# dangvansam/viet-asr

Hardware: AMD Instinct MI355X
Metric: real_time_factor (higher is better)
Workload: dtype f32 via 2xf16 split operands (22-bit significands, 3 f16 MFMA products per multiply, fp32 accumulate); 1 GPU; BASELINE configs[2]: quartznet15x5 greedy CTC, batch=64x10s 16kHz mono per GPU, wav in HBM -> collapsed ids; batch_per_gpu=64, parallelism=utterance-shard x1

## Files before the change

include/vasr_devtools.h:

```cpp
#ifndef VASR_DEVTOOLS_H_
#define VASR_DEVTOOLS_H_
#include "vasr.h"
#ifdef __cplusplus
extern "C" {
#endif

VASR_API int vasr_profile_bracket_overhead(vasr_stream stream, int n, double* out_us);
VASR_API int vasr_fused_tile_choice(int64_t tiles128, int compute_units);
VASR_API int vasr_bench_depthwise(const float* d_x, const float* d_w, const int32_t* d_lens, int batch, int channels,
                         int64_t frames, int kernel, float* d_y, vasr_stream stream);
VASR_API int vasr_bench_depthwise_layer(const float* d_x, const float* d_w, const int32_t* d_lens_in, const int32_t* d_lens_out,
                               int batch, int channels, int64_t frames_in, int kernel, int stride, int dilation, float* d_y,
                               uint32_t* d_amax, int amax_stride, vasr_stream stream);
VASR_API int vasr_depthwise_mfma_table_size(int kernel, int dilation);
VASR_API int vasr_pack_depthwise_taps(const float* h_w, int channels, int kernel, int dilation, uint32_t* h_table, float* h_inv);
VASR_API int vasr_bench_depthwise_mfma(const float* d_x, const uint32_t* d_taps, const float* d_tap_inv, const int32_t* d_lens,
                              int batch, int channels, int64_t frames, int kernel, int dilation, float* d_y,
                              uint32_t* d_amax, int amax_stride, vasr_stream stream);
VASR_API int vasr_pack_pointwise(const float* h_w, int cout, int cin, int m_pad, float* h_out);
VASR_API int vasr_conv_gemm_weights(const float* h_w, int cout, int cin, int kernel, float* h_out);
VASR_API int vasr_bench_pointwise(const float* d_x, const float* d_wt, const float* d_scale, const float* d_shift,
                         int batch, int cin, int cout, int64_t frames, float* d_y, vasr_stream stream);

VASR_API int vasr_bench_mfma_sustained(int gemm_mode, int workgroups, int steps, float* d_sink, double* flops, vasr_stream stream);
// ... 18 lines not shown
```

viet-asr_amd/_lib.py:

```python
import ctypes as C
import os

import numpy as np
import torch

_HERE = os.path.dirname(os.path.abspath(__file__))
LIB_PATH = os.environ.get("VASR_LIB_PATH") or os.path.join(_HERE, "lib", "libvasr_hip.so")
DEV_LIB_PATH = os.environ.get("VASR_LIB_PATH") or os.path.join(_HERE, "lib", "libvasr_hip_dev.so")


class VasrError(RuntimeError):
    pass


class BlockDesc(C.Structure):
    _fields_ = [(n, C.c_int32) for n in
                ("filters", "repeat", "kernel", "stride", "dilation", "residual", "separable", "residual_dense")]


class FrontendDesc(C.Structure):
    _fields_ = [("sample_rate", C.c_int32), ("n_fft", C.c_int32), ("win_length", C.c_int32),
                ("hop_length", C.c_int32), ("n_mels", C.c_int32), ("preemph", C.c_float),
                ("log_guard", C.c_float), ("normalize", C.c_int32),
                ("h_window", C.POINTER(C.c_float)), ("h_filterbank", C.POINTER(C.c_float)),
# ... 63 lines not shown
    "vasr_algorithmic_work": (C.c_int, [_P, C.c_int, C.c_int64, C.POINTER(C.c_double)]),
    "vasr_profile_begin": (C.c_int, [_P]),
    "vasr_profile_end": (C.c_int, [_P, C.POINTER(C.c_double), C.POINTER(C.c_int64), C.POINTER(C.c_double), C.POINTER(C.c_double)]),
    "vasr_padded_frames": (C.c_int64, [C.c_int64]),
}

DEV_SIGNATURES = {
    "vasr_pack_pointwise_f16x2": (C.c_int, [_P, C.c_int, C.c_int, C.c_int, _P, C.POINTER(C.c_float)]),
    "vasr_bench_pointwise_f16x2": (C.c_int, [_P, _P, C.c_float, _P, _P, C.c_int, C.c_int, C.c_int, C.c_int64, _P, _P,
                                             C.c_int, _P]),
    "vasr_depthwise_mfma_table_size": (C.c_int, [C.c_int, C.c_int]),
    "vasr_pack_depthwise_taps": (C.c_int, [_P, C.c_int, C.c_int, C.c_int, _P, _P]),
    "vasr_bench_depthwise_mfma": (C.c_int, [_P, _P, _P, _P, C.c_int, C.c_int, C.c_int64, C.c_int, C.c_int, _P, _P, C.c_int, _P]),
    "vasr_profile_bracket_overhead": (C.c_int, [_P, C.c_int, C.POINTER(C.c_double)]),
    "vasr_fused_tile_choice": (C.c_int, [C.c_int64, C.c_int]),
    "vasr_pack_pointwise": (C.c_int, [_P, C.c_int, C.c_int, C.c_int, _P]),
    "vasr_conv_gemm_weights": (C.c_int, [_P, C.c_int, C.c_int, C.c_int, _P]),
    "vasr_pack_pointwise_bf16x3": (C.c_int, [_P, C.c_int, C.c_int, C.c_int, _P]),
    "vasr_bench_pointwise_bf16x3": (C.c_int, [_P, _P, _P, _P, C.c_int, C.c_int, C.c_int, C.c_int64, _P, _P]),
    "vasr_bench_mfma_sustained": (C.c_int, [C.c_int, C.c_int, C.c_int, _P, C.POINTER(C.c_double), _P]),
    "vasr_bench_depthwise": (C.c_int, [_P, _P, _P, C.c_int, C.c_int, C.c_int64, C.c_int, _P, _P]),
    "vasr_bench_depthwise_layer": (C.c_int, [_P, _P, _P, _P, C.c_int, C.c_int, C.c_int64, C.c_int, C.c_int, C.c_int, _P, _P,
                                             C.c_int, _P]),
    "vasr_bench_pointwise": (C.c_int, [_P, _P, _P, _P, C.c_int, C.c_int, C.c_int, C.c_int64, _P, _P]),
    "vasr_bench_groupnorm": (C.c_int, [_P, _P, C.c_int, C.c_int, C.c_int64, C.c_int, C.c_int, _P, _P, C.c_int, _P, _P]),
}

ABI_VERSION = 8

_lib = None
# ... 175 lines not shown
```

viet-asr_amd/csrc/frontend.hip:

```cpp
#include <atomic>

#include "vasr_internal.h"
#include "len_chain.h"
#include "vasr_device.h"

namespace vasr {

namespace {

constexpr int kWaves = 8;
constexpr int kThreads = 64 * kWaves;
constexpr int kNfft = 512;

struct cf { float re, im; };
__device__ __forceinline__ cf cadd(cf a, cf b) { return {a.re + b.re, a.im + b.im}; }
__device__ __forceinline__ cf csub(cf a, cf b) { return {a.re - b.re, a.im - b.im}; }
__device__ __forceinline__ cf cmul(cf a, cf b) { return {a.re * b.re - a.im * b.im, a.re * b.im + a.im * b.re}; }
__device__ __forceinline__ cf cmul_negi(cf a) { return {a.im, -a.re}; }


__device__ __forceinline__ float sample_f32(const float* x, int64_t n) { return x[n]; }
__device__ __forceinline__ float sample_f32(const short* x, int64_t n) { return (float)x[n] * 0x1p-15f; }

template <int kFramesPerBlock, typename S>
__global__ __launch_bounds__(kThreads, 4) void stft_logmel_kernel(FrontendTables tb, const S* __restrict__ wav,
                                                          int64_t samples, const int64_t* __restrict__ row_len,
                                                          int hop, float preemph,
                                                          float log_guard, float* __restrict__ mel,
                                                          int64_t mel_ld, int frames) {
  constexpr int kFramesPerWave = kFramesPerBlock / kWaves;
  extern __shared__ __attribute__((aligned(16))) float smem[];
  const int seg_len = (kFramesPerBlock - 1) * hop + kNfft;
  float* seg = smem;
  cf* fftbuf = reinterpret_cast<cf*>(seg + ((seg_len + 3) & ~3));
  float* pbuf = reinterpret_cast<float*>(fftbuf + kWaves * 256);
  float* tile = pbuf + kWaves * (260 + kMelTaps);

  const int tid = threadIdx.x, lane = tid & 63, wave = tid >> 6;
  const int b = blockIdx.y;
  const int f0 = blockIdx.x * kFramesPerBlock;
  const S* x = wav + (int64_t)b * samples;
  const int64_t ns = row_len ? min(row_len[b], samples) : samples;

  const float2* win2 = reinterpret_cast<const float2*>(tb.window);
  const float2* t256 = reinterpret_cast<const float2*>(tb.tw256);
  const float2* t512 = reinterpret_cast<const float2*>(tb.tw512);
  float2 wn[4];
#pragma unroll
  for (int r = 0; r < 4; ++r) wn[r] = win2[lane + 64 * r];
  cf tws[3][3];
#pragma unroll
  for (int g = 0; g < 3; ++g) {
    const int Ns = 4 << (2 * g), step = (lane & (Ns - 1)) * (64 / Ns);
#pragma unroll
    for (int m = 0; m < 3; ++m) { const float2 w = t256[(m + 1) * step]; tws[g][m] = {w.x, w.y}; }
  }
  cf twk[5];
#pragma unroll
  for (int i = 0; i < 5; ++i) { const float2 w = t512[min(lane + 64 * i, 256)]; twk[i] = {w.x, w.y}; }
  const int64_t p0 = (int64_t)f0 * hop - kNfft / 2;
  for (int i = tid; i < seg_len; i += kThreads) {
    int64_t n = p0 + i;
    if (n < 0) n = -n;
    if (n >= ns) n = 2 * (ns - 1) - n;
    float v = 0.f;
    if (n >= 0 && n < ns) {
      v = sample_f32(x, n);
      if (preemph >= 0.f && n > 0) v = __fsub_rn(v, __fmul_rn(preemph, sample_f32(x, n - 1)));
    }
    seg[i] = v;
  }
  float mw[kMelTaps];
#pragma unroll
  for (int i = 0; i < kMelTaps; ++i) mw[i] = tb.mel_w[lane * kMelTaps + i];
  const int mlo = tb.mel_lo[lane];
  float* P = pbuf + wave * (260 + kMelTaps);
  for (int i = lane; i < 260 + kMelTaps; i += 64) P[i] = 0.f;
  __syncthreads();

  cf* buf = fftbuf + wave * 256;

  for (int jf = 0; jf < kFramesPerWave; ++jf) {
    const int fl = wave * kFramesPerWave + jf;
    const float* s = seg + fl * hop;
    {
      cf v[4];
#pragma unroll
      for (int r = 0; r < 4; ++r) {
        const int q = lane + 64 * r;
        v[r] = {s[2 * q] * wn[r].x, s[2 * q + 1] * wn[r].y};
      }
      cf t0 = cadd(v[0], v[2]), t1 = csub(v[0], v[2]), t2 = cadd(v[1], v[3]), t3 = cmul_negi(csub(v[1], v[3]));
      buf[4 * lane + 0] = cadd(t0, t2);
      buf[4 * lane + 1] = cadd(t1, t3);
      buf[4 * lane + 2] = csub(t0, t2);
      buf[4 * lane + 3] = csub(t1, t3);
    }
    wave_fence();
#pragma unroll
    for (int g = 0; g < 3; ++g) {
      const int Ns = 4 << (2 * g);
      const int k = lane & (Ns - 1);
      cf v[4];
#pragma unroll
      for (int r = 0; r < 4; ++r) v[r] = buf[lane + 64 * r];
      wave_fence();
      v[1] = cmul(v[1], tws[g][0]);
      v[2] = cmul(v[2], tws[g][1]);
      v[3] = cmul(v[3], tws[g][2]);
      cf t0 = cadd(v[0], v[2]), t1 = csub(v[0], v[2]), t2 = cadd(v[1], v[3]), t3 = cmul_negi(csub(v[1], v[3]));
      const int j0 = (lane / Ns) * Ns * 4 + k;
      buf[j0] = cadd(t0, t2);
      buf[j0 + Ns] = cadd(t1, t3);
      buf[j0 + 2 * Ns] = csub(t0, t2);
      buf[j0 + 3 * Ns] = csub(t1, t3);
      wave_fence();
    }
    const cf* Z = buf;
#pragma unroll
    for (int i = 0; i < 5; ++i) {
      const int k = lane + 64 * i;
      if (k > 256) break;
      cf zk = Z[k & 255];
      cf zc = Z[(256 - k) & 255];
      zc.im = -zc.im;
      cf e = {0.5f * (zk.re + zc.re), 0.5f * (zk.im + zc.im)};
      cf d = {zk.re - zc.re, zk.im - zc.im};
      cf o = {0.5f * d.im, -0.5f * d.re};
      cf xk = cadd(e, cmul(twk[i], o));
      P[k] = xk.re * xk.re + xk.im * xk.im;
    }
    wave_fence();
    float acc = 0.f;
#pragma unroll
    for (int i = 0; i < kMelTaps; ++i) acc = fmaf(mw[i], P[mlo + i], acc);
    tile[lane * (kFramesPerBlock + 1) + fl] = tb.guard_clamp ? logf(fmaxf(acc, log_guard)) : logf(acc + log_guard);
    wave_fence();
  }
  __syncthreads();
  for (int idx = tid; idx < 64 * kFramesPerBlock; idx += kThreads) {
    const int f = idx / kFramesPerBlock, j = idx % kFramesPerBlock;
    const int t = f0 + j;
    if (t < frames) mel[((int64_t)b * 64 + f) * mel_ld + t] = tile[f * (kFramesPerBlock + 1) + j];
  }
}

__global__ void seq_len_kernel(const int64_t* __restrict__ len, int batch, int hop, int64_t* __restrict__ seq) {
  const int b = blockIdx.x * blockDim.x + threadIdx.x;
  if (b < batch) seq[b] = (int64_t)ceilf((float)len[b] / (float)hop);
}

__device__ __forceinline__ double wave_sum(double v) {
#pragma unroll
  for (int o = 32; o > 0; o >>= 1) v += __shfl_xor(v, o, 64);
  return v;
}

__device__ __forceinline__ int64_t seq_of(int64_t len, int hop) { return (int64_t)ceilf((float)len / (float)hop); }

constexpr int kRowsPerWg = 4;
__device__ __forceinline__ void normalize_row(float* __restrict__ x, int n, int frames, int normalize, double* red) {
  const int tid = threadIdx.x & 255, lane = tid & 63, wv = tid >> 6;
  float mean = 0.f, stdv = 1.f;
  if (normalize) {
    double s = 0.0;
    for (int t = tid; t < n; t += 256) s += (double)x[t];
    s = wave_sum(s);
    if (lane == 0) red[wv] = s;
    __syncthreads();
    const double mu = (((red[0] + red[1]) + red[2]) + red[3]) / (double)n;
    double q = 0.0;
    for (int t = tid; t < n; t += 256) { const double d = (double)x[t] - mu; q += d * d; }
    q = wave_sum(q);
    if (lane == 0) red[4 + wv] = q;
    __syncthreads();
    mean = (float)mu;
    stdv = (float)sqrt((((red[4] + red[5]) + red[6]) + red[7]) / (double)(n - 1));
    stdv = stdv + 1e-5f;
  }
  for (int t = tid; t < frames; t += 256) {
    float v = 0.f;
    if (t < n) v = normalize ? (x[t] - mean) / stdv : x[t];
    x[t] = v;
  }
}

__global__ __launch_bounds__(256 * kRowsPerWg) void normalize_kernel(float* __restrict__ mel, int64_t ld,
                                                                     const int64_t* __restrict__ seq, int rows, int n_mels,
                                                                     int frames, int normalize) {
  __shared__ double red[kRowsPerWg][8];
  const int grp = threadIdx.x >> 8;
  const int row = min((int)blockIdx.x * kRowsPerWg + grp, rows - 1);
  const int64_t n64 = seq[row / n_mels];
  normalize_row(mel + (int64_t)row * ld, (int)(n64 < 0 ? 0 : (n64 > frames ? frames : n64)), frames, normalize, red[grp]);
}

__global__ __launch_bounds__(256) void normalize_all_kernel(float* __restrict__ mel, int64_t ld, const int64_t* __restrict__ seq,
                                                            int n_mels, int frames) {
  __shared__ double red[8];
  const int tid = threadIdx.x, lane = tid & 63, wv = tid >> 6;
  float* x = mel + (int64_t)blockIdx.x * n_mels * ld;
  const int64_t n64 = seq[blockIdx.x];
  const int n = (int)(n64 < 0 ? 0 : (n64 > frames ? frames : n64));
  const double cnt = (double)n * (double)n_mels;
  double s = 0.0;
  for (int f = 0; f < n_mels; ++f)
    for (int t = tid; t < n; t += 256) s += (double)x[(int64_t)f * ld + t];
  s = wave_sum(s);
  if (lane == 0) red[wv] = s;
// ... 4 lines not shown
    for (int t = tid; t < n; t += 256) { const double d = (double)x[(int64_t)f * ld + t] - mu; q += d * d; }
  q = wave_sum(q);
  if (lane == 0) red[4 + wv] = q;
  __syncthreads();
  const float mean = (float)mu;
  const float stdv = (float)sqrt((((red[4] + red[5]) + red[6]) + red[7]) / (cnt - 1.0)) + 1e-5f;
  for (int f = 0; f < n_mels; ++f)
    for (int t = tid; t < n; t += 256) x[(int64_t)f * ld + t] = (x[(int64_t)f * ld + t] - mean) / stdv;
}

__global__ __launch_bounds__(256 * kRowsPerWg) void normalize_chain_kernel(float* __restrict__ mel, int64_t ld,
                                                              const int64_t* __restrict__ len, int hop, int batch, int n_mels,
                                                              int frames, int normalize, int64_t* __restrict__ seq,
                                                              const LenStep* __restrict__ steps, int n_steps,
                                                              int32_t* __restrict__ lens_tab, float* __restrict__ enc_len,
                                                              const int64_t* __restrict__ wav_len, int frames_cap) {
  __shared__ double red[kRowsPerWg][8];
  const int rows = batch * n_mels, row_wgs = (rows + kRowsPerWg - 1) / kRowsPerWg;
  if ((int)blockIdx.x < row_wgs) {
    const int grp = threadIdx.x >> 8;
    const int row = min((int)blockIdx.x * kRowsPerWg + grp, rows - 1);
    const int64_t n64 = seq_of(len[row / n_mels], hop);
    normalize_row(mel + (int64_t)row * ld, (int)(n64 < 0 ? 0 : (n64 > frames ? frames : n64)), frames, normalize, red[grp]);
    return;
  }
  const int b = ((int)blockIdx.x - row_wgs) * 256 * kRowsPerWg + (int)threadIdx.x;
  const int64_t l0 = b < batch ? seq_of(len[b], hop) : 0;
  if (b < batch) seq[b] = l0;
  len_chain_body(b, l0, batch, steps, n_steps, lens_tab, enc_len, wav_len, hop, frames_cap);
}

}

void launch_stft_logmel(const FrontendTables& tb, const void* wav, bool pcm16, int batch, int64_t samples,
                        const int64_t* row_len, int hop, float preemph, float log_guard, float* mel, int64_t mel_ld, int frames,
                        hipStream_t st) {
  auto go = [&](auto kern, auto* wav, int fpb) {
    const int seg_len = (fpb - 1) * hop + kNfft;
    const size_t lds = (size_t)((seg_len + 3) & ~3) * 4 + kWaves * 256 * 8 + kWaves * (260 + kMelTaps) * 4 + 64 * (fpb + 1) * 4;
    dim3 grid((frames + fpb - 1) / fpb, batch);
    hipLaunchKernelGGL(kern, grid, dim3(kThreads), lds, st, tb, wav, samples, row_len, hop, preemph, log_guard, mel, mel_ld,
                       frames);
  };
  const bool small = (int64_t)((frames + 31) / 32) * batch < 128;
  if (pcm16) {
    if (small) go(stft_logmel_kernel<8, short>, static_cast<const short*>(wav), 8);
    else go(stft_logmel_kernel<32, short>, static_cast<const short*>(wav), 32);
  } else {
    if (small) go(stft_logmel_kernel<8, float>, static_cast<const float*>(wav), 8);
    else go(stft_logmel_kernel<32, float>, static_cast<const float*>(wav), 32);
  }
}

void launch_seq_len(const int64_t* len, int batch, int hop, int64_t* seq, hipStream_t st) {
  hipLaunchKernelGGL(seq_len_kernel, dim3((batch + 63) / 64), dim3(64), 0, st, len, batch, hop, seq);
}

constexpr int kAloneLds = 152 * 1024;

void launch_normalize_all(float* mel, int64_t mel_ld, const int64_t* seq, int batch, int n_mels, int frames, hipStream_t st) {
  static std::atomic<uint64_t> opted{0};
  (void)dyn_lds_opt_in(reinterpret_cast<const void*>(normalize_all_kernel), kAloneLds, opted);
  hipLaunchKernelGGL(normalize_all_kernel, dim3(batch), dim3(256), kAloneLds, st, mel, mel_ld, seq, n_mels, frames);
}

void launch_normalize(float* mel, int64_t mel_ld, const int64_t* seq, int batch, int n_mels, int frames,
                      int normalize, hipStream_t st) {
  const int rows = batch * n_mels;
  static std::atomic<uint64_t> opted{0};
  (void)dyn_lds_opt_in(reinterpret_cast<const void*>(normalize_kernel), kAloneLds, opted);
  hipLaunchKernelGGL(normalize_kernel, dim3((rows + kRowsPerWg - 1) / kRowsPerWg), dim3(256 * kRowsPerWg), normalize ? kAloneLds : 0, st, mel, mel_ld,
                     seq, rows, n_mels, frames, normalize);
}

void launch_normalize_chain(float* mel, int64_t mel_ld, const int64_t* len, int hop, int batch, int n_mels, int frames,
                            int normalize, int64_t* seq, const LenStep* d_steps, int n_steps, int32_t* lens_tab,
                            float* enc_len, const int64_t* wav_len, int frames_cap, hipStream_t st) {
  const int rows = batch * n_mels;
  static std::atomic<uint64_t> opted{0};
  (void)dyn_lds_opt_in(reinterpret_cast<const void*>(normalize_chain_kernel), kAloneLds, opted);
  const int wg = 256 * kRowsPerWg;
  hipLaunchKernelGGL(normalize_chain_kernel, dim3((rows + kRowsPerWg - 1) / kRowsPerWg + (batch + wg - 1) / wg), dim3(wg), normalize ? kAloneLds : 0, st, mel, mel_ld, len, hop, batch,
                     n_mels, frames, normalize, seq, d_steps, n_steps, lens_tab, enc_len, wav_len, frames_cap);
}

}
```

viet-asr_amd/csrc/vasr_api.cpp:

```cpp
#include <hip/hip_runtime.h>

#include <cmath>
#include <cstdarg>
#include <cstdio>
#include <cstdlib>
#include <cstring>
#include <map>
#include <memory>
#include <string>
#include <algorithm>
#include <vector>

#include "vasr.h"
#include "vasr_host.h"
#include "vasr_internal.h"

using namespace vasr;

namespace {
thread_local std::string g_err;
}

namespace vasr {

// ... 1321 lines not shown
  return whole;
}

int vasr_melspec_f32(vasr_handle* h, const float* d_wav, const int64_t* d_len, int batch, int64_t samples,
                     float* d_mel, int64_t* d_seq, vasr_stream stream) {
  if (!h || !h->has_frontend || !h->finalized) return fail(VASR_ERR_STATE, "no finalized front end in this handle");
  if (batch <= 0 || !d_wav || !d_len || !d_mel || !d_seq) return fail(VASR_ERR_INVALID, "bad argument");
  if (samples <= h->fe.n_fft / 2)
    return fail(VASR_ERR_INVALID, "reflect padding needs more than n_fft/2 = %d samples (got %lld)",
                h->fe.n_fft / 2, (long long)samples);
  hipStream_t st = static_cast<hipStream_t>(stream);
  const int T = (int)vasr_mel_frames(h, samples);
  launch_seq_len(d_len, batch, h->fe.hop_length, d_seq, st);
  launch_stft_logmel(h->ft, d_wav, false, batch, samples, h->row_independent ? d_len : nullptr, h->fe.hop_length,
                     h->fe.preemph, h->fe.log_guard, d_mel, T, T, st);
  launch_normalize(d_mel, T, d_seq, batch, h->fe.n_mels, T, h->fe.normalize == 1, st);
  if (h->fe.normalize == 2) launch_normalize_all(d_mel, T, d_seq, batch, h->fe.n_mels, T, st);
  return check_launch("melspec");
}

int vasr_encoder_f32(vasr_handle* h, const float* d_mel, const int64_t* d_seq, int batch, int64_t mel_frames,
                     float* d_enc, float* d_enc_len, void* d_ws, size_t ws_bytes, vasr_stream stream) {
  if (!h || !h->has_encoder || !h->finalized) return fail(VASR_ERR_STATE, "no finalized encoder in this handle");
  if (batch <= 0 || mel_frames <= 0 || !d_mel || !d_seq || !d_enc || !d_ws) return fail(VASR_ERR_INVALID, "bad argument");
  const WsPlan p = plan_ws(h, batch, mel_frames);
  if (ws_bytes < p.total) return fail(VASR_ERR_WORKSPACE, "workspace %zu < %zu bytes", ws_bytes, p.total);
  hipStream_t st = static_cast<hipStream_t>(stream);
  char* ws = static_cast<char*>(d_ws);
  const Block& b0 = h->blocks[0];
  if (b0.subs[0].separable && !b0.has_res)
    return run_encoder(h, d_mel, mel_frames, mel_frames, d_seq, batch, d_enc, p.T1, d_enc_len, ws, p, st);
// ... 131 lines not shown

static int transcribe_part(vasr_handle* h, const void* d_wav, bool pcm16, const int64_t* d_len, int batch, int64_t samples,
                           int64_t* d_pred, int32_t* d_ids, int32_t* d_id_len, float* d_logp, float* d_enc_len,
                           char* ws, hipStream_t st) {
  const int64_t T = vasr_mel_frames(h, samples);
  const WsPlan p = plan_ws(h, batch, T);
  int64_t* seq = reinterpret_cast<int64_t*>(ws + p.seq);
  float* melp = reinterpret_cast<float*>(ws + p.melp);
  float* encp = reinterpret_cast<float*>(ws + p.encp);
  float* logits = reinterpret_cast<float*>(ws + p.logits);
  int64_t* pred = d_pred ? d_pred : reinterpret_cast<int64_t*>(ws + p.pred);
  {
    ProfScope ps(h, kProfFrontend, st);
    launch_stft_logmel(h->ft, d_wav, pcm16, batch, samples, h->row_independent ? d_len : nullptr, h->fe.hop_length,
                       h->fe.preemph, h->fe.log_guard, melp, p.Tp0, (int)T, st);
    launch_normalize_chain(melp, p.Tp0, d_len, h->fe.hop_length, batch, h->fe.n_mels, (int)T, h->fe.normalize == 1, seq,
                           h->d_steps, (int)h->steps.size(), reinterpret_cast<int32_t*>(ws + p.lens_tab), d_enc_len,
                           h->row_independent ? d_len : nullptr, (int)p.T1, st);
    if (h->fe.normalize == 2) launch_normalize_all(melp, p.Tp0, seq, batch, h->fe.n_mels, (int)T, st);
  }
  AmaxTab enc_amax{};
  const int32_t* own_frames = nullptr;
  int rc = run_encoder(h, melp, p.Tp0, T, seq, batch, encp, p.Tp1, d_enc_len, ws, p, st, &enc_amax, d_len, &own_frames, true);
  if (rc) return rc;
  if ((rc = run_decoder(h, encp, p.Tp1, p.T1, batch, logits, d_logp, pred, st, enc_amax, own_frames))) return rc;
  if (d_ids && d_id_len) {
    ProfScope ps(h, kProfHead, st);
    if (h->row_independent)
      launch_ctc_collapse(pred, batch, p.T1, h->num_classes - 1, d_ids, d_id_len, st, d_len, h->fe.hop_length,
                          h->d_steps, (int)h->steps.size());
    else
      launch_ctc_collapse(pred, batch, p.T1, h->num_classes - 1, d_ids, d_id_len, st);
  }
// ... 152 lines not shown
    return fail(VASR_ERR_INVALID, "%lld mel frames are cropped to %lld: offsets needed", (long long)c.T, (long long)audio_length);
  if (ws_bytes < c.total) return fail(VASR_ERR_WORKSPACE, "workspace %zu < %zu bytes", ws_bytes, c.total);
  hipStream_t st = static_cast<hipStream_t>(stream);
  char* ws = static_cast<char*>(d_ws);
  const WsPlan& p = c.enc;
  float* mel_raw = reinterpret_cast<float*>(ws + c.mel_raw);
  int64_t* seq_raw = reinterpret_cast<int64_t*>(ws + c.seq_raw);
  int64_t* seq = reinterpret_cast<int64_t*>(ws + p.seq);
  float* melp = reinterpret_cast<float*>(ws + p.melp);
  float* encp = reinterpret_cast<float*>(ws + p.encp);
  {
    ProfScope ps(h, kProfFrontend, st);
    launch_seq_len(d_len, batch, h->fe.hop_length, seq_raw, st);
    launch_stft_logmel(h->ft, d_wav, false, batch, samples, h->row_independent ? d_len : nullptr, h->fe.hop_length,
                       h->fe.preemph, h->fe.log_guard, mel_raw, c.Tp, (int)c.T, st);
    launch_normalize(mel_raw, c.Tp, seq_raw, batch, h->fe.n_mels, (int)c.T, h->fe.normalize == 1, st);
    if (h->fe.normalize == 2) launch_normalize_all(mel_raw, c.Tp, seq_raw, batch, h->fe.n_mels, (int)c.T, st);
    const int e = launch_crop_or_pad(mel_raw, c.Tp, batch, h->fe.n_mels, (int)c.T, h->row_independent ? d_len : nullptr,
                                     h->fe.hop_length, (int)audio_length, d_offsets, melp, p.Tp0, (int)p.Tp0, seq, st);
    if (e) return fail(VASR_ERR_HIP, "crop_or_pad: %s", hipGetErrorString((hipError_t)e));
    if (d_mel) launch_repad(melp, p.Tp0, batch * h->fe.n_mels, (int)audio_length, d_mel, audio_length, st);
  }
  int rc = run_encoder(h, melp, p.Tp0, audio_length, seq, batch, encp, p.Tp1, reinterpret_cast<float*>(ws + c.enc_len), ws, p, st);
  if (rc) return rc;
  if ((rc = run_classifier(h, encp, p.Tp1, p.T1, batch, softmax, reinterpret_cast<float*>(ws + c.pooled), d_out, st))) return rc;
  return check_launch("classify");
}

int vasr_pcm16_to_f32(const int16_t* d_pcm, int64_t n, float* d_out, vasr_stream stream) {
  if (!d_pcm || !d_out || n < 0) return fail(VASR_ERR_INVALID, "bad argument");
  if (n == 0) return 0;
// ... 201 lines not shown
```

viet-asr_amd/csrc/vasr_devtools.cpp:

```cpp
#include <hip/hip_runtime.h>

#include <algorithm>
#include <cstdio>
#include <cstdlib>
#include <initializer_list>
#include <vector>

#include "vasr.h"
#include "vasr_devtools.h"
#include "vasr_host.h"
#include "vasr_internal.h"

using namespace vasr;

const vasr::DevSwitches& vasr::dev_switches() {
  static const DevSwitches sw = [] {
    DevSwitches s;
    auto num = [](const char* name, int dflt, std::initializer_list<int> allowed) {
      const char* e = getenv(name);
      if (!e) return dflt;
      const int v = atoi(e);
      for (int a : allowed) if (a == v) return v;
      fprintf(stderr, "vasr (devtools build): %s=%s is not a documented value -- refusing to guess\n", name, e);
      abort();
      return dflt;
    };
    s.pw3_tile = num("VASR_PW3_TILE", 0, {0, 1, 2, 3, 4, 5});
    s.pw_lat = num("VASR_PW_LAT", 1, {0, 1});
    s.dw_pair = num("VASR_DW_PAIR", 1, {0, 1}) != 0;
    s.dw_mfma = num("VASR_DW_MFMA", 1, {0, 1}) != 0;
    s.dw_upw = num("VASR_DW_UPW", 0, {0, 1, 2, 3, 4, 5, 6, 7, 8});
    s.fused = num("VASR_FUSED", 1, {0, 1}) != 0;
    s.fused_min_tiles = getenv("VASR_FUSED_MIN_TILES") ? atoi(getenv("VASR_FUSED_MIN_TILES")) : 0;
    s.fused_tile = num("VASR_FUSED_TILE", 0, {0, 64, 128});
    s.fused_residual = num("VASR_NO_FUSED_RESIDUAL", 0, {0, 1}) == 0;
    s.beam_group = num("VASR_BEAM_GROUP", -1, {-1, 0, 1, 4});
    s.no_grouped = num("VASR_NO_GROUPED", 0, {0, 1}) != 0;
    return s;
  }();
  return sw;
}

extern "C" {

int vasr_fused_tile_choice(int64_t tiles128, int compute_units) { return vasr::fused_tile_choice(tiles128, compute_units); }

static __global__ void dev_noop_kernel() {}

int vasr_profile_bracket_overhead(vasr_stream stream, int n, double* out_us) {
  if (n < 1 || n > 4096 || !out_us) return fail(VASR_ERR_INVALID, "bad argument");
  hipStream_t st = static_cast<hipStream_t>(stream);
  std::vector<hipEvent_t> ev(2 * (size_t)n);
  for (auto& e : ev) HIP_TRY(hipEventCreate(&e));
  for (int i = 0; i < n; ++i) {
    HIP_TRY(hipEventRecord(ev[2 * i], st));
    hipLaunchKernelGGL(dev_noop_kernel, dim3(1), dim3(64), 0, st);
    HIP_TRY(hipEventRecord(ev[2 * i + 1], st));
  }
  HIP_TRY(hipEventSynchronize(ev.back()));
  std::vector<float> t(n);
// ... 182 lines not shown
```

viet-asr_amd/csrc/vasr_internal.h:

```cpp
#pragma once
#include <hip/hip_runtime.h>
#include <atomic>
#include <hip/hip_ext.h>
#include <stdint.h>
#include <stdlib.h>

namespace vasr {

struct DevSwitches {
  int pw3_tile = 0;
  int pw_lat = 1;
  bool dw_pair = true;
  bool dw_mfma = true;
  int dw_upw = 0;
  bool fused = true;
  int fused_min_tiles = 0;
  int fused_tile = 0;
  bool fused_residual = true;
  int beam_group = -1;
  bool no_grouped = false;
};
#ifdef VASR_DEVTOOLS
const DevSwitches& dev_switches();
#else
inline const DevSwitches& dev_switches() { static constexpr DevSwitches k{}; return k; }
#endif

struct LaunchProbe { hipEvent_t start = nullptr, stop = nullptr; };
extern thread_local LaunchProbe g_probe;
#define VASR_LAUNCH(kern, grid, block, lds, st, ...)                                                       \
  do {                                                                                                     \
    if (::vasr::g_probe.start) {                                                                           \
      hipExtLaunchKernelGGL(kern, grid, block, lds, st, ::vasr::g_probe.start, ::vasr::g_probe.stop, 0,   \
                            __VA_ARGS__);                                                                  \
      ::vasr::g_probe.start = nullptr;                                                                     \
// ... 35 lines not shown

struct FrontendTables {
  const float* window;
  const float* tw256;
  const float* tw512;
  const float* mel_w;
  const int32_t* mel_lo;
  int32_t guard_clamp;
};
constexpr int kMelTaps = 32;

void launch_stft_logmel(const FrontendTables& tb, const void* wav, bool pcm16, int batch, int64_t samples,
                        const int64_t* row_len, int hop, float preemph, float log_guard, float* mel, int64_t mel_ld, int frames,
                        hipStream_t st);
void launch_seq_len(const int64_t* len, int batch, int hop, int64_t* seq, hipStream_t st);
void launch_normalize_all(float* mel, int64_t mel_ld, const int64_t* seq, int batch, int n_mels, int frames, hipStream_t st);
void launch_normalize(float* mel, int64_t mel_ld, const int64_t* seq, int batch, int n_mels, int frames,
                      int normalize, hipStream_t st);

struct LenStep { int32_t kernel, stride, dilation, pad; };
void launch_normalize_chain(float* mel, int64_t mel_ld, const int64_t* len, int hop, int batch, int n_mels, int frames,
                            int normalize, int64_t* seq, const LenStep* d_steps, int n_steps, int32_t* lens_tab,
                            float* enc_len, const int64_t* wav_len, int frames_cap, hipStream_t st);
void launch_len_chain(const int64_t* seq, int batch, const LenStep* d_steps, int n_steps, int32_t* lens_tab,
                      float* enc_len, hipStream_t st, const int64_t* wav_len = nullptr, int hop = 1, int frames_cap = 0);

void launch_repad(const float* src, int64_t src_ld, int rows, int frames, float* dst, int64_t dst_ld,
                  hipStream_t st);

int launch_depthwise(const float* x, int64_t ldx, int frames_in, const float* w, const int32_t* lens_in,
                     const int32_t* lens_out, int batch, int channels, int kernel, int stride, int dilation,
                     int pad, float* y, int64_t ldy, hipStream_t st, AmaxTab* amax_y = nullptr);
int depthwise_amax_slots(int channels, int64_t ldy);

int depthwise_mfma_table_size(int kernel, int dilation);
float pack_depthwise_taps_f16x2(const float* w, int kernel, int dilation, int tsz, unsigned int* table);
int launch_depthwise_mfma(const float* x, int64_t ldx, const unsigned int* taps, const float* tap_inv,
                          const int32_t* lens_in, const int32_t* lens_out, AmaxTab amax_x, int batch,
// ... 186 lines not shown
```

Before: 124,200 audio-sec/wall-sec.

## Process two STFT frames per wave and hold normalize rows in registers

The STFT/log-mel kernel gains a two-frames-in-flight variant. Each wave interleaves the radix-4 FFT stages of two frames in separate LDS buffers, and the segment load batches eleven global loads per thread before use. Per-row normalization now keeps up to 4096 frames in registers, so it reads the mel row once instead of three times. The frontend is a small part of total time, and the extra LDS and registers could lower occupancy. Launch functions now return LDS opt-in errors, and a devtools switch and query select the old paths.

```diff
diff --git a/include/vasr_devtools.h b/include/vasr_devtools.h
--- a/include/vasr_devtools.h
+++ b/include/vasr_devtools.h
@@ -7,6 +7,7 @@
 
 VASR_API int vasr_profile_bracket_overhead(vasr_stream stream, int n, double* out_us);
 VASR_API int vasr_fused_tile_choice(int64_t tiles128, int compute_units);
+VASR_API int vasr_frontend_forms(int batch, int64_t frames, int hop, int fe_v1, int* normalize_form, int* stft_form);
 VASR_API int vasr_bench_depthwise(const float* d_x, const float* d_w, const int32_t* d_lens, int batch, int channels,
                          int64_t frames, int kernel, float* d_y, vasr_stream stream);
 VASR_API int vasr_bench_depthwise_layer(const float* d_x, const float* d_w, const int32_t* d_lens_in, const int32_t* d_lens_out,
diff --git a/viet-asr_amd/_lib.py b/viet-asr_amd/_lib.py
--- a/viet-asr_amd/_lib.py
+++ b/viet-asr_amd/_lib.py
@@ -101,6 +101,7 @@
     "vasr_bench_depthwise_mfma": (C.c_int, [_P, _P, _P, _P, C.c_int, C.c_int, C.c_int64, C.c_int, C.c_int, _P, _P, C.c_int, _P]),
     "vasr_profile_bracket_overhead": (C.c_int, [_P, C.c_int, C.POINTER(C.c_double)]),
     "vasr_fused_tile_choice": (C.c_int, [C.c_int64, C.c_int]),
+    "vasr_frontend_forms": (C.c_int, [C.c_int, C.c_int64, C.c_int, C.c_int, C.POINTER(C.c_int), C.POINTER(C.c_int)]),
     "vasr_pack_pointwise": (C.c_int, [_P, C.c_int, C.c_int, C.c_int, _P]),
     "vasr_conv_gemm_weights": (C.c_int, [_P, C.c_int, C.c_int, C.c_int, _P]),
     "vasr_pack_pointwise_bf16x3": (C.c_int, [_P, C.c_int, C.c_int, C.c_int, _P]),
diff --git a/viet-asr_amd/csrc/frontend.hip b/viet-asr_amd/csrc/frontend.hip
--- a/viet-asr_amd/csrc/frontend.hip
+++ b/viet-asr_amd/csrc/frontend.hip
@@ -11,6 +11,7 @@
 constexpr int kWaves = 8;
 constexpr int kThreads = 64 * kWaves;
 constexpr int kNfft = 512;
+static_assert(kNfft == 512 && kWaves == 8, "stft_lds_bytes (vasr_internal.h) sizes the LDS for these");
 
 struct cf { float re, im; };
 __device__ __forceinline__ cf cadd(cf a, cf b) { return {a.re + b.re, a.im + b.im}; }
@@ -19,10 +20,12 @@
 __device__ __forceinline__ cf cmul_negi(cf a) { return {a.im, -a.re}; }
 
 
-__device__ __forceinline__ float sample_f32(const float* x, int64_t n) { return x[n]; }
-__device__ __forceinline__ float sample_f32(const short* x, int64_t n) { return (float)x[n] * 0x1p-15f; }
-
-template <int kFramesPerBlock, typename S>
+__device__ __forceinline__ float sample_f32(float s) { return s; }
+__device__ __forceinline__ float sample_f32(short s) { return (float)s * 0x1p-15f; }
+__device__ __forceinline__ float sample_f32(const float* x, int64_t n) { return sample_f32(x[n]); }
+__device__ __forceinline__ float sample_f32(const short* x, int64_t n) { return sample_f32(x[n]); }
+
+template <int kFramesPerBlock, typename S, int kInFlight>
 __global__ __launch_bounds__(kThreads, 4) void stft_logmel_kernel(FrontendTables tb, const S* __restrict__ wav,
                                                           int64_t samples, const int64_t* __restrict__ row_len,
                                                           int hop, float preemph,
@@ -33,8 +36,8 @@
   const int seg_len = (kFramesPerBlock - 1) * hop + kNfft;
   float* seg = smem;
   cf* fftbuf = reinterpret_cast<cf*>(seg + ((seg_len + 3) & ~3));
-  float* pbuf = reinterpret_cast<float*>(fftbuf + kWaves * 256);
-  float* tile = pbuf + kWaves * (260 + kMelTaps);
+  float* pbuf = reinterpret_cast<float*>(fftbuf + kWaves * kInFlight * 256);
+  float* tile = pbuf + (kInFlight == 1 ? kWaves * (260 + kMelTaps) : 0);
 
   const int tid = threadIdx.x, lane = tid & 63, wave = tid >> 6;
   const int b = blockIdx.y;
@@ -59,83 +62,202 @@
 #pragma unroll
   for (int i = 0; i < 5; ++i) { const float2 w = t512[min(lane + 64 * i, 256)]; twk[i] = {w.x, w.y}; }
   const int64_t p0 = (int64_t)f0 * hop - kNfft / 2;
-  for (int i = tid; i < seg_len; i += kThreads) {
-    int64_t n = p0 + i;
-    if (n < 0) n = -n;
-    if (n >= ns) n = 2 * (ns - 1) - n;
-    float v = 0.f;
-    if (n >= 0 && n < ns) {
-      v = sample_f32(x, n);
-      if (preemph >= 0.f && n > 0) v = __fsub_rn(v, __fmul_rn(preemph, sample_f32(x, n - 1)));
-    }
-    seg[i] = v;
+  if constexpr (kInFlight > 1) {
+    constexpr int kStage = 11;
+    for (int i0 = tid; i0 < seg_len; i0 += kThreads * kStage) {
+      S cur[kStage], prv[kStage];
+#pragma unroll
+      for (int u = 0; u < kStage; ++u) {
+        int64_t n = p0 + i0 + u * kThreads;
+        if (n < 0) n = -n;
+        if (n >= ns) n = 2 * (ns - 1) - n;
+        const int64_t nc = min(max(n, (int64_t)0), samples - 1);
+        cur[u] = x[nc];
+        prv[u] = x[max(nc - 1, (int64_t)0)];
+      }
+#pragma unroll
+      for (int u = 0; u < kStage; ++u) {
+        int64_t n = p0 + i0 + u * kThreads;
+        if (n < 0) n = -n;
+        if (n >= ns) n = 2 * (ns - 1) - n;
+        float v = 0.f;
+        if (n >= 0 && n < ns) {
+          v = sample_f32(cur[u]);
+          if (preemph >= 0.f && n > 0) v = fmaf(-preemph, sample_f32(prv[u]), v);
+        }
+        if (i0 + u * kThreads < seg_len) seg[i0 + u * kThreads] = v;
+      }
+    }
+  } else {
+    for (int i = tid; i < seg_len; i += kThreads) {
+      int64_t n = p0 + i;
+      if (n < 0) n = -n;
+      if (n >= ns) n = 2 * (ns - 1) - n;
+      float v = 0.f;
+      if (n >= 0 && n < ns) {
+        v = sample_f32(x, n);
+        if (preemph >= 0.f && n > 0) v = __fsub_rn(v, __fmul_rn(preemph, sample_f32(x, n - 1)));
+      }
+      seg[i] = v;
+    }
   }
   float mw[kMelTaps];
 #pragma unroll
   for (int i = 0; i < kMelTaps; ++i) mw[i] = tb.mel_w[lane * kMelTaps + i];
   const int mlo = tb.mel_lo[lane];
   float* P = pbuf + wave * (260 + kMelTaps);
-  for (int i = lane; i < 260 + kMelTaps; i += 64) P[i] = 0.f;
+  if constexpr (kInFlight == 1)
+    for (int i = lane; i < 260 + kMelTaps; i += 64) P[i] = 0.f;
   __syncthreads();
 
   cf* buf = fftbuf + wave * 256;
 
-  for (int jf = 0; jf < kFramesPerWave; ++jf) {
-    const int fl = wave * kFramesPerWave + jf;
-    const float* s = seg + fl * hop;
-    {
-      cf v[4];
-#pragma unroll
-      for (int r = 0; r < 4; ++r) {
-        const int q = lane + 64 * r;
-        v[r] = {s[2 * q] * wn[r].x, s[2 * q + 1] * wn[r].y};
-      }
-      cf t0 = cadd(v[0], v[2]), t1 = csub(v[0], v[2]), t2 = cadd(v[1], v[3]), t3 = cmul_negi(csub(v[1], v[3]));
-      buf[4 * lane + 0] = cadd(t0, t2);
-      buf[4 * lane + 1] = cadd(t1, t3);
-      buf[4 * lane + 2] = csub(t0, t2);
-      buf[4 * lane + 3] = csub(t1, t3);
-    }
-    wave_fence();
-#pragma unroll
-    for (int g = 0; g < 3; ++g) {
-      const int Ns = 4 << (2 * g);
-      const int k = lane & (Ns - 1);
-      cf v[4];
-#pragma unroll
-      for (int r = 0; r < 4; ++r) v[r] = buf[lane + 64 * r];
-      wave_fence();
-      v[1] = cmul(v[1], tws[g][0]);
-      v[2] = cmul(v[2], tws[g][1]);
-      v[3] = cmul(v[3], tws[g][2]);
-      cf t0 = cadd(v[0], v[2]), t1 = csub(v[0], v[2]), t2 = cadd(v[1], v[3]), t3 = cmul_negi(csub(v[1], v[3]));
-      const int j0 = (lane / Ns) * Ns * 4 + k;
-      buf[j0] = cadd(t0, t2);
-      buf[j0 + Ns] = cadd(t1, t3);
-      buf[j0 + 2 * Ns] = csub(t0, t2);
-      buf[j0 + 3 * Ns] = csub(t1, t3);
-      wave_fence();
-    }
-    const cf* Z = buf;
-#pragma unroll
-    for (int i = 0; i < 5; ++i) {
-      const int k = lane + 64 * i;
-      if (k > 256) break;
-      cf zk = Z[k & 255];
-      cf zc = Z[(256 - k) & 255];
-      zc.im = -zc.im;
-      cf e = {0.5f * (zk.re + zc.re), 0.5f * (zk.im + zc.im)};
-      cf d = {zk.re - zc.re, zk.im - zc.im};
-      cf o = {0.5f * d.im, -0.5f * d.re};
-      cf xk = cadd(e, cmul(twk[i], o));
-      P[k] = xk.re * xk.re + xk.im * xk.im;
-    }
-    wave_fence();
-    float acc = 0.f;
-#pragma unroll
-    for (int i = 0; i < kMelTaps; ++i) acc = fmaf(mw[i], P[mlo + i], acc);
-    tile[lane * (kFramesPerBlock + 1) + fl] = tb.guard_clamp ? logf(fmaxf(acc, log_guard)) : logf(acc + log_guard);
-    wave_fence();
+  if constexpr (kInFlight > 1) {
+    static_assert(kInFlight == 2 && kFramesPerWave % 2 == 0, "two frames in flight");
+    cf* bufs[2] = {fftbuf + (wave * 2) * 256, fftbuf + (wave * 2 + 1) * 256};
+    for (int jf = 0; jf < kFramesPerWave; jf += 2) {
+      const int fl0 = wave * kFramesPerWave + jf;
+      cf v[2][4];
+#pragma unroll
+      for (int u = 0; u < 2; ++u) {
+        const float* s = seg + (fl0 + u) * hop;
+#pragma unroll
+        for (int r = 0; r < 4; ++r) {
+          const int q = lane + 64 * r;
+          v[u][r] = {s[2 * q] * wn[r].x, s[2 * q + 1] * wn[r].y};
+        }
+      }
+#pragma unroll
+      for (int u = 0; u < 2; ++u) {
+        cf t0 = cadd(v[u][0], v[u][2]), t1 = csub(v[u][0], v[u][2]), t2 = cadd(v[u][1], v[u][3]),
+           t3 = cmul_negi(csub(v[u][1], v[u][3]));
+        bufs[u][4 * lane + 0] = cadd(t0, t2);
+        bufs[u][4 * lane + 1] = cadd(t1, t3);
+        bufs[u][4 * lane + 2] = csub(t0, t2);
+        bufs[u][4 * lane + 3] = csub(t1, t3);
+      }
+      wave_fence();
+#pragma unroll
+      for (int g = 0; g < 3; ++g) {
+        const int Ns = 4 << (2 * g);
+        const int k = lane & (Ns - 1);
+#pragma unroll
+        for (int u = 0; u < 2; ++u)
+#pragma unroll
+          for (int r = 0; r < 4; ++r) v[u][r] = bufs[u][lane + 64 * r];
+        wave_fence();
+        const int j0 = (lane / Ns) * Ns * 4 + k;
+#pragma unroll
+        for (int u = 0; u < 2; ++u) {
+          v[u][1] = cmul(v[u][1], tws[g][0]);
+          v[u][2] = cmul(v[u][2], tws[g][1]);
+          v[u][3] = cmul(v[u][3], tws[g][2]);
+          cf t0 = cadd(v[u][0], v[u][2]), t1 = csub(v[u][0], v[u][2]), t2 = cadd(v[u][1], v[u][3]),
+             t3 = cmul_negi(csub(v[u][1], v[u][3]));
+          bufs[u][j0] = cadd(t0, t2);
+          bufs[u][j0 + Ns] = cadd(t1, t3);
+          bufs[u][j0 + 2 * Ns] = csub(t0, t2);
+          bufs[u][j0 + 3 * Ns] = csub(t1, t3);
+        }
+        wave_fence();
+      }
+      float pw[2][5];
+#pragma unroll
+      for (int u = 0; u < 2; ++u) {
+        const cf* Z = bufs[u];
+#pragma unroll
+        for (int i = 0; i < 5; ++i) {
+          const int k = lane + 64 * i;
+          cf zk = Z[k & 255];
+          cf zc = Z[(256 - k) & 255];
+          zc.im = -zc.im;
+          cf e = {0.5f * (zk.re + zc.re), 0.5f * (zk.im + zc.im)};
+          cf d = {zk.re - zc.re, zk.im - zc.im};
+          cf o = {0.5f * d.im, -0.5f * d.re};
+          cf xk = cadd(e, cmul(twk[i], o));
+          pw[u][i] = xk.re * xk.re + xk.im * xk.im;
+        }
+      }
+      wave_fence();
+#pragma unroll
+      for (int u = 0; u < 2; ++u) {
+        float* Pu = reinterpret_cast<float*>(bufs[u]);
+#pragma unroll
+        for (int i = 0; i < 5; ++i) {
+          const int k = lane + 64 * i;
+          if (k <= 256) Pu[k] = pw[u][i];
+        }
+        if (lane < 3 + kMelTaps) Pu[257 + lane] = 0.f;
+      }
+      wave_fence();
+#pragma unroll
+      for (int u = 0; u < 2; ++u) {
+        const float* Pu = reinterpret_cast<const float*>(bufs[u]);
+        float acc = 0.f;
+#pragma unroll
+        for (int i = 0; i < kMelTaps; ++i) acc = fmaf(mw[i], Pu[mlo + i], acc);
+        tile[lane * (kFramesPerBlock + 1) + fl0 + u] = tb.guard_clamp ? logf(fmaxf(acc, log_guard)) : logf(acc + log_guard);
+      }
+      wave_fence();
+    }
+  } else {
+    for (int jf = 0; jf < kFramesPerWave; ++jf) {
+      const int fl = wave * kFramesPerWave + jf;
+      const float* s = seg + fl * hop;
+      {
+        cf v[4];
+  #pragma unroll
+        for (int r = 0; r < 4; ++r) {
+          const int q = lane + 64 * r;
+          v[r] = {s[2 * q] * wn[r].x, s[2 * q + 1] * wn[r].y};
+        }
+        cf t0 = cadd(v[0], v[2]), t1 = csub(v[0], v[2]), t2 = cadd(v[1], v[3]), t3 = cmul_negi(csub(v[1], v[3]));
+        buf[4 * lane + 0] = cadd(t0, t2);
+        buf[4 * lane + 1] = cadd(t1, t3);
+        buf[4 * lane + 2] = csub(t0, t2);
+        buf[4 * lane + 3] = csub(t1, t3);
+      }
+      wave_fence();
+  #pragma unroll
+      for (int g = 0; g < 3; ++g) {
+        const int Ns = 4 << (2 * g);
+        const int k = lane & (Ns - 1);
+        cf v[4];
+  #pragma unroll
+        for (int r = 0; r < 4; ++r) v[r] = buf[lane + 64 * r];
+        wave_fence();
+        v[1] = cmul(v[1], tws[g][0]);
+        v[2] = cmul(v[2], tws[g][1]);
+        v[3] = cmul(v[3], tws[g][2]);
+        cf t0 = cadd(v[0], v[2]), t1 = csub(v[0], v[2]), t2 = cadd(v[1], v[3]), t3 = cmul_negi(csub(v[1], v[3]));
+        const int j0 = (lane / Ns) * Ns * 4 + k;
+        buf[j0] = cadd(t0, t2);
+        buf[j0 + Ns] = cadd(t1, t3);
+        buf[j0 + 2 * Ns] = csub(t0, t2);
+        buf[j0 + 3 * Ns] = csub(t1, t3);
+        wave_fence();
+      }
+      const cf* Z = buf;
+  #pragma unroll
+      for (int i = 0; i < 5; ++i) {
+        const int k = lane + 64 * i;
+        if (k > 256) break;
+        cf zk = Z[k & 255];
+        cf zc = Z[(256 - k) & 255];
+        zc.im = -zc.im;
+        cf e = {0.5f * (zk.re + zc.re), 0.5f * (zk.im + zc.im)};
+        cf d = {zk.re - zc.re, zk.im - zc.im};
+        cf o = {0.5f * d.im, -0.5f * d.re};
+        cf xk = cadd(e, cmul(twk[i], o));
+        P[k] = xk.re * xk.re + xk.im * xk.im;
+      }
+      wave_fence();
+      float acc = 0.f;
+  #pragma unroll
+      for (int i = 0; i < kMelTaps; ++i) acc = fmaf(mw[i], P[mlo + i], acc);
+      tile[lane * (kFramesPerBlock + 1) + fl] = tb.guard_clamp ? logf(fmaxf(acc, log_guard)) : logf(acc + log_guard);
+      wave_fence();
+    }
   }
   __syncthreads();
   for (int idx = tid; idx < 64 * kFramesPerBlock; idx += kThreads) {
@@ -159,9 +281,45 @@
 __device__ __forceinline__ int64_t seq_of(int64_t len, int hop) { return (int64_t)ceilf((float)len / (float)hop); }
 
 constexpr int kRowsPerWg = 4;
-__device__ __forceinline__ void normalize_row(float* __restrict__ x, int n, int frames, int normalize, double* red) {
+__device__ __forceinline__ void normalize_row(float* __restrict__ x, int n, int frames, int normalize, int regs, double* red) {
   const int tid = threadIdx.x & 255, lane = tid & 63, wv = tid >> 6;
   float mean = 0.f, stdv = 1.f;
+  if (regs) {
+    float xr[kNormRegs];
+#pragma unroll
+    for (int i = 0; i < kNormRegs; ++i)
+      if (256 * i < frames) { const int t = tid + 256 * i; xr[i] = t < n ? x[t] : 0.f; }
+    if (normalize) {
+      double s = 0.0;
+#pragma unroll
+      for (int i = 0; i < kNormRegs; ++i)
+        if (256 * i < frames && tid + 256 * i < n) s += (double)xr[i];
+      s = wave_sum(s);
+      if (lane == 0) red[wv] = s;
+      __syncthreads();
+      const double mu = (((red[0] + red[1]) + red[2]) + red[3]) / (double)n;
+      double q = 0.0;
+#pragma unroll
+      for (int i = 0; i < kNormRegs; ++i)
+        if (256 * i < frames && tid + 256 * i < n) { const double d = (double)xr[i] - mu; q += d * d; }
+      q = wave_sum(q);
+      if (lane == 0) red[4 + wv] = q;
+      __syncthreads();
+      mean = (float)mu;
+      stdv = (float)sqrt((((red[4] + red[5]) + red[6]) + red[7]) / (double)(n - 1));
+      stdv = stdv + 1e-5f;
+    }
+#pragma unroll
+    for (int i = 0; i < kNormRegs; ++i) {
+      const int t = tid + 256 * i;
+      if (256 * i < frames && t < frames) {
+        float v = 0.f;
+        if (t < n) v = normalize ? (xr[i] - mean) / stdv : xr[i];
+        x[t] = v;
+      }
+    }
+    return;
+  }
   if (normalize) {
     double s = 0.0;
     for (int t = tid; t < n; t += 256) s += (double)x[t];
@@ -187,12 +345,12 @@
 
 __global__ __launch_bounds__(256 * kRowsPerWg) void normalize_kernel(float* __restrict__ mel, int64_t ld,
                                                                      const int64_t* __restrict__ seq, int rows, int n_mels,
-                                                                     int frames, int normalize) {
+                                                                     int frames, int normalize, int regs) {
   __shared__ double red[kRowsPerWg][8];
   const int grp = threadIdx.x >> 8;
   const int row = min((int)blockIdx.x * kRowsPerWg + grp, rows - 1);
   const int64_t n64 = seq[row / n_mels];
-  normalize_row(mel + (int64_t)row * ld, (int)(n64 < 0 ? 0 : (n64 > frames ? frames : n64)), frames, normalize, red[grp]);
+  normalize_row(mel + (int64_t)row * ld, (int)(n64 < 0 ? 0 : (n64 > frames ? frames : n64)), frames, normalize, regs, red[grp]);
 }
 
 __global__ __launch_bounds__(256) void normalize_all_kernel(float* __restrict__ mel, int64_t ld, const int64_t* __restrict__ seq,
@@ -227,14 +385,14 @@
                                                               int frames, int normalize, int64_t* __restrict__ seq,
                                                               const LenStep* __restrict__ steps, int n_steps,
                                                               int32_t* __restrict__ lens_tab, float* __restrict__ enc_len,
-                                                              const int64_t* __restrict__ wav_len, int frames_cap) {
+                                                              const int64_t* __restrict__ wav_len, int frames_cap, int regs) {
   __shared__ double red[kRowsPerWg][8];
   const int rows = batch * n_mels, row_wgs = (rows + kRowsPerWg - 1) / kRowsPerWg;
   if ((int)blockIdx.x < row_wgs) {
     const int grp = threadIdx.x >> 8;
     const int row = min((int)blockIdx.x * kRowsPerWg + grp, rows - 1);
     const int64_t n64 = seq_of(len[row / n_mels], hop);
-    normalize_row(mel + (int64_t)row * ld, (int)(n64 < 0 ? 0 : (n64 > frames ? frames : n64)), frames, normalize, red[grp]);
+    normalize_row(mel + (int64_t)row * ld, (int)(n64 < 0 ? 0 : (n64 > frames ? frames : n64)), frames, normalize, regs, red[grp]);
     return;
   }
   const int b = ((int)blockIdx.x - row_wgs) * 256 * kRowsPerWg + (int)threadIdx.x;
@@ -248,20 +406,22 @@
 void launch_stft_logmel(const FrontendTables& tb, const void* wav, bool pcm16, int batch, int64_t samples,
                         const int64_t* row_len, int hop, float preemph, float log_guard, float* mel, int64_t mel_ld, int frames,
                         hipStream_t st) {
-  auto go = [&](auto kern, auto* wav, int fpb) {
-    const int seg_len = (fpb - 1) * hop + kNfft;
-    const size_t lds = (size_t)((seg_len + 3) & ~3) * 4 + kWaves * 256 * 8 + kWaves * (260 + kMelTaps) * 4 + 64 * (fpb + 1) * 4;
+  auto go = [&](auto kern, auto* wav, int fpb, int in_flight) {
     dim3 grid((frames + fpb - 1) / fpb, batch);
-    hipLaunchKernelGGL(kern, grid, dim3(kThreads), lds, st, tb, wav, samples, row_len, hop, preemph, log_guard, mel, mel_ld,
-                       frames);
+    hipLaunchKernelGGL(kern, grid, dim3(kThreads), stft_lds_bytes(fpb, in_flight, hop), st, tb, wav, samples, row_len, hop, preemph,
+                       log_guard, mel, mel_ld, frames);
   };
-  const bool small = (int64_t)((frames + 31) / 32) * batch < 128;
+  const int form = stft_form(batch, frames, hop, dev_switches().fe_v1);
   if (pcm16) {
-    if (small) go(stft_logmel_kernel<8, short>, static_cast<const short*>(wav), 8);
-    else go(stft_logmel_kernel<32, short>, static_cast<const short*>(wav), 32);
+    const short* w = static_cast<const short*>(wav);
+    if (form == kStftSmall) go(stft_logmel_kernel<8, short, 1>, w, 8, 1);
+    else if (form == kStftSerial) go(stft_logmel_kernel<32, short, 1>, w, 32, 1);
+    else go(stft_logmel_kernel<32, short, 2>, w, 32, 2);
   } else {
-    if (small) go(stft_logmel_kernel<8, float>, static_cast<const float*>(wav), 8);
-    else go(stft_logmel_kernel<32, float>, static_cast<const float*>(wav), 32);
+    const float* w = static_cast<const float*>(wav);
+    if (form == kStftSmall) go(stft_logmel_kernel<8, float, 1>, w, 8, 1);
+    else if (form == kStftSerial) go(stft_logmel_kernel<32, float, 1>, w, 32, 1);
+    else go(stft_logmel_kernel<32, float, 2>, w, 32, 2);
   }
 }
 
@@ -277,24 +437,28 @@
   hipLaunchKernelGGL(normalize_all_kernel, dim3(batch), dim3(256), kAloneLds, st, mel, mel_ld, seq, n_mels, frames);
 }
 
-void launch_normalize(float* mel, int64_t mel_ld, const int64_t* seq, int batch, int n_mels, int frames,
-                      int normalize, hipStream_t st) {
+int launch_normalize(float* mel, int64_t mel_ld, const int64_t* seq, int batch, int n_mels, int frames,
+                     int normalize, hipStream_t st) {
   const int rows = batch * n_mels;
   static std::atomic<uint64_t> opted{0};
-  (void)dyn_lds_opt_in(reinterpret_cast<const void*>(normalize_kernel), kAloneLds, opted);
+  if (const hipError_t e = dyn_lds_opt_in(reinterpret_cast<const void*>(normalize_kernel), kAloneLds, opted)) return (int)e;
+  const int regs = normalize_form(frames, dev_switches().fe_v1) == kNormalizeRegs;
   hipLaunchKernelGGL(normalize_kernel, dim3((rows + kRowsPerWg - 1) / kRowsPerWg), dim3(256 * kRowsPerWg), normalize ? kAloneLds : 0, st, mel, mel_ld,
-                     seq, rows, n_mels, frames, normalize);
-}
-
-void launch_normalize_chain(float* mel, int64_t mel_ld, const int64_t* len, int hop, int batch, int n_mels, int frames,
-                            int normalize, int64_t* seq, const LenStep* d_steps, int n_steps, int32_t* lens_tab,
-                            float* enc_len, const int64_t* wav_len, int frames_cap, hipStream_t st) {
+                     seq, rows, n_mels, frames, normalize, regs);
+  return 0;
+}
+
+int launch_normalize_chain(float* mel, int64_t mel_ld, const int64_t* len, int hop, int batch, int n_mels, int frames,
+                           int normalize, int64_t* seq, const LenStep* d_steps, int n_steps, int32_t* lens_tab,
+                           float* enc_len, const int64_t* wav_len, int frames_cap, hipStream_t st) {
   const int rows = batch * n_mels;
   static std::atomic<uint64_t> opted{0};
-  (void)dyn_lds_opt_in(reinterpret_cast<const void*>(normalize_chain_kernel), kAloneLds, opted);
+  if (const hipError_t e = dyn_lds_opt_in(reinterpret_cast<const void*>(normalize_chain_kernel), kAloneLds, opted)) return (int)e;
   const int wg = 256 * kRowsPerWg;
+  const int regs = normalize_form(frames, dev_switches().fe_v1) == kNormalizeRegs;
   hipLaunchKernelGGL(normalize_chain_kernel, dim3((rows + kRowsPerWg - 1) / kRowsPerWg + (batch + wg - 1) / wg), dim3(wg), normalize ? kAloneLds : 0, st, mel, mel_ld, len, hop, batch,
-                     n_mels, frames, normalize, seq, d_steps, n_steps, lens_tab, enc_len, wav_len, frames_cap);
-}
-
-}
+                     n_mels, frames, normalize, seq, d_steps, n_steps, lens_tab, enc_len, wav_len, frames_cap, regs);
+  return 0;
+}
+
+}
diff --git a/viet-asr_amd/csrc/vasr_api.cpp b/viet-asr_amd/csrc/vasr_api.cpp
--- a/viet-asr_amd/csrc/vasr_api.cpp
+++ b/viet-asr_amd/csrc/vasr_api.cpp
@@ -1359,7 +1359,8 @@
   launch_seq_len(d_len, batch, h->fe.hop_length, d_seq, st);
   launch_stft_logmel(h->ft, d_wav, false, batch, samples, h->row_independent ? d_len : nullptr, h->fe.hop_length,
                      h->fe.preemph, h->fe.log_guard, d_mel, T, T, st);
-  launch_normalize(d_mel, T, d_seq, batch, h->fe.n_mels, T, h->fe.normalize == 1, st);
+  if (const int e = launch_normalize(d_mel, T, d_seq, batch, h->fe.n_mels, T, h->fe.normalize == 1, st))
+    return fail(VASR_ERR_HIP, "normalize: dynamic LDS opt-in: %s", hipGetErrorString((hipError_t)e));
   if (h->fe.normalize == 2) launch_normalize_all(d_mel, T, d_seq, batch, h->fe.n_mels, T, st);
   return check_launch("melspec");
 }
@@ -1521,9 +1522,11 @@
     ProfScope ps(h, kProfFrontend, st);
     launch_stft_logmel(h->ft, d_wav, pcm16, batch, samples, h->row_independent ? d_len : nullptr, h->fe.hop_length,
                        h->fe.preemph, h->fe.log_guard, melp, p.Tp0, (int)T, st);
-    launch_normalize_chain(melp, p.Tp0, d_len, h->fe.hop_length, batch, h->fe.n_mels, (int)T, h->fe.normalize == 1, seq,
-                           h->d_steps, (int)h->steps.size(), reinterpret_cast<int32_t*>(ws + p.lens_tab), d_enc_len,
-                           h->row_independent ? d_len : nullptr, (int)p.T1, st);
+    if (const int e = launch_normalize_chain(melp, p.Tp0, d_len, h->fe.hop_length, batch, h->fe.n_mels, (int)T,
+                                             h->fe.normalize == 1, seq, h->d_steps, (int)h->steps.size(),
+                                             reinterpret_cast<int32_t*>(ws + p.lens_tab), d_enc_len,
+                                             h->row_independent ? d_len : nullptr, (int)p.T1, st))
+      return fail(VASR_ERR_HIP, "normalize: dynamic LDS opt-in: %s", hipGetErrorString((hipError_t)e));
     if (h->fe.normalize == 2) launch_normalize_all(melp, p.Tp0, seq, batch, h->fe.n_mels, (int)T, st);
   }
   AmaxTab enc_amax{};
@@ -1706,7 +1709,8 @@
     launch_seq_len(d_len, batch, h->fe.hop_length, seq_raw, st);
     launch_stft_logmel(h->ft, d_wav, false, batch, samples, h->row_independent ? d_len : nullptr, h->fe.hop_length,
                        h->fe.preemph, h->fe.log_guard, mel_raw, c.Tp, (int)c.T, st);
-    launch_normalize(mel_raw, c.Tp, seq_raw, batch, h->fe.n_mels, (int)c.T, h->fe.normalize == 1, st);
+    if (const int e = launch_normalize(mel_raw, c.Tp, seq_raw, batch, h->fe.n_mels, (int)c.T, h->fe.normalize == 1, st))
+      return fail(VASR_ERR_HIP, "normalize: dynamic LDS opt-in: %s", hipGetErrorString((hipError_t)e));
     if (h->fe.normalize == 2) launch_normalize_all(mel_raw, c.Tp, seq_raw, batch, h->fe.n_mels, (int)c.T, st);
     const int e = launch_crop_or_pad(mel_raw, c.Tp, batch, h->fe.n_mels, (int)c.T, h->row_independent ? d_len : nullptr,
                                      h->fe.hop_length, (int)audio_length, d_offsets, melp, p.Tp0, (int)p.Tp0, seq, st);
diff --git a/viet-asr_amd/csrc/vasr_devtools.cpp b/viet-asr_amd/csrc/vasr_devtools.cpp
--- a/viet-asr_amd/csrc/vasr_devtools.cpp
+++ b/viet-asr_amd/csrc/vasr_devtools.cpp
@@ -36,6 +36,7 @@
     s.fused_residual = num("VASR_NO_FUSED_RESIDUAL", 0, {0, 1}) == 0;
     s.beam_group = num("VASR_BEAM_GROUP", -1, {-1, 0, 1, 4});
     s.no_grouped = num("VASR_NO_GROUPED", 0, {0, 1}) != 0;
+    s.fe_v1 = num("VASR_FE_V1", 0, {0, 1}) != 0;
     return s;
   }();
   return sw;
@@ -44,6 +45,13 @@
 extern "C" {
 
 int vasr_fused_tile_choice(int64_t tiles128, int compute_units) { return vasr::fused_tile_choice(tiles128, compute_units); }
+
+int vasr_frontend_forms(int batch, int64_t frames, int hop, int fe_v1, int* normalize_form, int* stft_form) {
+  if (batch < 1 || frames < 1 || hop < 1 || !normalize_form || !stft_form) return fail(VASR_ERR_INVALID, "bad argument");
+  *normalize_form = vasr::normalize_form(frames, fe_v1 != 0);
+  *stft_form = vasr::stft_form(batch, frames, hop, fe_v1 != 0);
+  return 0;
+}
 
 static __global__ void dev_noop_kernel() {}
 
diff --git a/viet-asr_amd/csrc/vasr_internal.h b/viet-asr_amd/csrc/vasr_internal.h
--- a/viet-asr_amd/csrc/vasr_internal.h
+++ b/viet-asr_amd/csrc/vasr_internal.h
@@ -19,6 +19,7 @@
   bool fused_residual = true;
   int beam_group = -1;
   bool no_grouped = false;
+  bool fe_v1 = false;
 };
 #ifdef VASR_DEVTOOLS
 const DevSwitches& dev_switches();
@@ -84,14 +85,26 @@
                         const int64_t* row_len, int hop, float preemph, float log_guard, float* mel, int64_t mel_ld, int frames,
                         hipStream_t st);
 void launch_seq_len(const int64_t* len, int batch, int hop, int64_t* seq, hipStream_t st);
+constexpr int kNormRegs = 16;
+enum : int { kNormalizeRegs = 0, kNormalizeLoop = 1 };
+inline int normalize_form(int64_t frames, bool fe_v1) { return !fe_v1 && frames <= 256 * kNormRegs ? kNormalizeRegs : kNormalizeLoop; }
+enum : int { kStftSmall = 0, kStftTwoInFlight = 1, kStftSerial = 2 };
+inline size_t stft_lds_bytes(int frames_per_wg, int in_flight, int hop) {
+  return (size_t)(((frames_per_wg - 1) * hop + 512 + 3) & ~3) * 4 + (size_t)8 * in_flight * 256 * 8 +
+         (in_flight == 1 ? (size_t)8 * (260 + kMelTaps) * 4 : 0) + (size_t)64 * (frames_per_wg + 1) * 4;
+}
+inline int stft_form(int batch, int64_t frames, int hop, bool fe_v1) {
+  if ((frames + 31) / 32 * batch < 128) return kStftSmall;
+  return !fe_v1 && stft_lds_bytes(32, 2, hop) <= 64 * 1024 ? kStftTwoInFlight : kStftSerial;
+}
 void launch_normalize_all(float* mel, int64_t mel_ld, const int64_t* seq, int batch, int n_mels, int frames, hipStream_t st);
-void launch_normalize(float* mel, int64_t mel_ld, const int64_t* seq, int batch, int n_mels, int frames,
-                      int normalize, hipStream_t st);
+int launch_normalize(float* mel, int64_t mel_ld, const int64_t* seq, int batch, int n_mels, int frames,
+                     int normalize, hipStream_t st);
 
 struct LenStep { int32_t kernel, stride, dilation, pad; };
-void launch_normalize_chain(float* mel, int64_t mel_ld, const int64_t* len, int hop, int batch, int n_mels, int frames,
-                            int normalize, int64_t* seq, const LenStep* d_steps, int n_steps, int32_t* lens_tab,
-                            float* enc_len, const int64_t* wav_len, int frames_cap, hipStream_t st);
+int launch_normalize_chain(float* mel, int64_t mel_ld, const int64_t* len, int hop, int batch, int n_mels, int frames,
+                           int normalize, int64_t* seq, const LenStep* d_steps, int n_steps, int32_t* lens_tab,
+                           float* enc_len, const int64_t* wav_len, int frames_cap, hipStream_t st);
 void launch_len_chain(const int64_t* seq, int batch, const LenStep* d_steps, int n_steps, int32_t* lens_tab,
                       float* enc_len, hipStream_t st, const int64_t* wav_len = nullptr, int hop = 1, int frames_cap = 0);
 
```

Result: no change. 124,700 audio-sec/wall-sec (median of 6 runs) (+0.4%).
